# su1phurd/UAV-WRF-LES-PPO-LSTM

Hardware: AMD Instinct MI355X
Metric: env-steps/sec (rollout + GAE + 5-epoch PPO update), 4096 envs x 128 T per GPU, LSTM h=128 x1 (higher is better)
Workload: dtype f32

## Files before the change

### uav-wrf-les-ppo-lstm_amd/csrc/lstm.hip

```cpp
#include <stdlib.h>
#include <type_traits>
#include "common.h"

int gemm_f32(uav_ctx* ctx, int64_t M, int64_t N, int64_t K, const float* A, int64_t sa_m, int64_t sa_k,
             const float* B, int64_t sb_k, int64_t sb_n, float* C, int64_t ldc, const float* bias,
             int accumulate, hipStream_t st);
int colsum(uav_ctx* ctx, const float* X, int64_t B, int C, float* out, float* scratch, hipStream_t st);
int colsum_absmax(uav_ctx* ctx, const float* X, int64_t B, int C, float* out, float* scratch, unsigned* absmax_bits,
                  hipStream_t st);
int colsum_xw(uav_ctx* ctx, const float* X, int64_t B, int C, const float* x, int I, float* colsum_out, float* xw_out,
              float* scratch, unsigned* absmax_bits, hipStream_t st, int xw_transposed = 0);
bool gemm_h3_ok(int64_t M, int64_t N, int64_t K, const float* A, int64_t sa_m, int64_t sa_k, const float* B, int64_t sb_k,
                int64_t sb_n);
int gemm_h3(uav_ctx* ctx, int64_t M, int64_t N, int64_t K, const float* A, int64_t sa_m, int64_t sa_k, const float* B,
            int64_t sb_k, int64_t sb_n, float* C, int64_t ldc, const float* bias, int accumulate, const unsigned* a_absmax,
            hipStream_t st);
int lstm_generic_fwd(uav_ctx* ctx, const float* keep, const float* h0, const float* c0, const float* w_hh, int N, int T,
                     int H, float* y, float* hn, float* cn, float* stash, hipStream_t st);
int lstm_h3_fwd(uav_ctx* ctx, const float* x, int I, const float* w_ih, const float* b_ih, const float* b_hh,
                const float* keep, const float* h0, const float* c0, const float* w_hh, int N, int T, float* y, float* hn,
                float* cn, float* stash, hipStream_t st);
bool lstm_h3_step_path(int H);
int lstm_generic_bwd(uav_ctx* ctx, const float* keep, const float* stash, const float* w_hh, const float* dy,
                     const float* dheads, const float* w_head, int n_heads,
// ... 101 lines not shown
            const int t = t0 + tt;
            f32x4 acc[4];
#pragma unroll
            for (int q = 0; q < 4; ++q) {
                if (FUSE_X) {
                    acc[q] = f32x4{bias[q], bias[q], bias[q], bias[q]};
                } else {
#pragma unroll
                    for (int r = 0; r < 4; ++r) {
                        const int n = min(n0 + 4 * kq + r, N - 1);
                        acc[q][r] = stash[((size_t)n * T + t) * (6 * H) + q * H + u];
                    }
                }
            }
            if (FUSE_X) {
                const float2 ax = *reinterpret_cast<const float2*>(&xbuf[(tt * MT + j) * 8 + 2 * kq]);
#pragma unroll
                for (int q = 0; q < 4; ++q) {
                    acc[q] = __builtin_amdgcn_mfma_f32_16x16x4f32(ax.x, wx[q][0], acc[q], 0, 0, 0);
                    acc[q] = __builtin_amdgcn_mfma_f32_16x16x4f32(ax.y, wx[q][1], acc[q], 0, 0, 0);
                }
            }
            const float* hrow = hbuf + cur * MT * S + j * S + kq * SEG;
#pragma unroll
            for (int s = 0; s < KS; s += 4) {
                const float4 a = *reinterpret_cast<const float4*>(hrow + s);
#pragma unroll
                for (int q = 0; q < 4; ++q) acc[q] = __builtin_amdgcn_mfma_f32_16x16x4f32(a.x, wh[q][s], acc[q], 0, 0, 0);
#pragma unroll
                for (int q = 0; q < 4; ++q) acc[q] = __builtin_amdgcn_mfma_f32_16x16x4f32(a.y, wh[q][s + 1], acc[q], 0, 0, 0);
#pragma unroll
                for (int q = 0; q < 4; ++q) acc[q] = __builtin_amdgcn_mfma_f32_16x16x4f32(a.z, wh[q][s + 2], acc[q], 0, 0, 0);
#pragma unroll
                for (int q = 0; q < 4; ++q) acc[q] = __builtin_amdgcn_mfma_f32_16x16x4f32(a.w, wh[q][s + 3], acc[q], 0, 0, 0);
            }
            float* hnext = hbuf + (cur ^ 1) * MT * S;
#pragma unroll
            for (int r = 0; r < 4; ++r) {
                const int e = 4 * kq + r;
                const int n = n0 + e;
                const float gi = sigmoidf_(acc[0][r]), gf = sigmoidf_(acc[1][r]);
                const float gg = tanhf_(acc[2][r]), go = sigmoidf_(acc[3][r]);
                const float cp = c_reg[r];
                const float c = gf * cp + gi * gg;
                const float h = go * tanhf_(c);
                const float kn = kbuf[(tt + 1) * MT + e];
                if (n < N) {
                    const size_t row = (size_t)n * T + t;
                    y[row * H + u] = h;
                    if (stash) {
                        float* sp = stash + row * (6 * H);
                        sp[u] = gi; sp[H + u] = gf; sp[2 * H + u] = gg; sp[3 * H + u] = go;
                        sp[4 * H + u] = cp;
                        if (I > 6) sp[5 * H + u] = hin[r];
                    }
                }
                h_last[r] = h;
                if (t == T - 1) c_reg[r] = c;
                else c_reg[r] = c * kn;
                hin[r] = h * kn;
                hnext[e * S + hpos<H>(u)] = hin[r];
            }
            cur ^= 1;
            lds_barrier();
        }
    }
#pragma unroll
    for (int r = 0; r < 4; ++r) {
        const int n = n0 + 4 * kq + r;
        if (n < N) {
            hn[(size_t)n * H + u] = h_last[r];
            cn[(size_t)n * H + u] = c_reg[r];
        }
    }
}

template <class P, int H>
struct FwdSplitGeom {
    static constexpr int NS = H / 32;
    static constexpr int RS = H + 8;
    static constexpr int PLANE = MT * RS;
    static constexpr int QL = P::fwd_park(H);
    static constexpr int WPARK = QL * NS * 64 * 8;
    static constexpr int TCX = 8;
    static constexpr int XPT = (MT * TCX * 8 + H * 4 - 1) / (H * 4);
    static constexpr int HPL = 8 * RS;
    static constexpr size_t LDS = (2 * P::NP * PLANE + (H / 16) * WPARK + P::NP * HPL) * sizeof(unsigned short) +
                                  (2 * TCX * MT * 8 + 2 * TCX * MT + (H / 16) * 8 * 64 + 4 * H + 8) * sizeof(float);
};
#ifdef UAV_X6_PROFILE
__device__ unsigned long long g_x6_prof[2][8];
#define X6_PROF_DECL unsigned long long pm_[8] = {0, 0, 0, 0, 0, 0, 0, 0}, pl_ = __builtin_readcyclecounter()
#define X6_PROF_MARK(i) do { const unsigned long long n_ = __builtin_readcyclecounter(); pm_[i] += n_ - pl_; pl_ = n_; } while (0)
#define X6_PROF_DEP(v) asm volatile("" ::"v"(v))
#define X6_PROF_FLUSH() do { if (blockIdx.x == 0 && lane == 0 && (w == 0 || w == H / 16 - 1)) \
        for (int i_ = 0; i_ < 4; ++i_) g_x6_prof[w ? 1 : 0][i_] = pm_[i_]; } while (0)
#define X6_PROF_FLUSH8() do { if (blockIdx.x == 0 && lane == 0 && (w == 0 || w == H / 16 - 1)) \
        for (int i_ = 0; i_ < 8; ++i_) g_x6_prof[w ? 1 : 0][i_] = pm_[i_]; } while (0)
extern "C" int uav_x6_prof_read(unsigned long long* out) {
    return hipMemcpyFromSymbol(out, HIP_SYMBOL(g_x6_prof), sizeof(g_x6_prof)) == hipSuccess ? 0 : 1;
}
#else
#define X6_PROF_DECL
#define X6_PROF_MARK(i)
#define X6_PROF_DEP(v)
#define X6_PROF_FLUSH()
#define X6_PROF_FLUSH8()
#endif

template <class P, int H, bool FUSE_X>
__device__ __forceinline__ void lstm_fwd_split(
    const float* __restrict__ x, const float* __restrict__ keep, const float* __restrict__ h0,
    const float* __restrict__ c0, const float* __restrict__ w_ih, const float* __restrict__ w_hh,
    const float* __restrict__ b_ih, const float* __restrict__ b_hh, int N, int T, int I,
    float* __restrict__ y, float* __restrict__ hn, float* __restrict__ cn, float* __restrict__ stash,
    const float* __restrict__ w_head, const float* __restrict__ b_head, int NHD, float* __restrict__ heads) {
    using G = FwdSplitGeom<P, H>;
    using vec = typename P::vec;
    using piece = typename P::piece;
    constexpr int NP = P::NP, NS = G::NS, RS = G::RS, PLANE = G::PLANE, QL = G::QL, WPARK = G::WPARK, TC = G::TCX;
    constexpr int XPT = G::XPT, NT = H * 4, HPL = G::HPL, NW = H / 16;
    extern __shared__ __attribute__((aligned(16))) float smem[];
    unsigned short* hpl = reinterpret_cast<unsigned short*>(smem);
    unsigned short* wpark = hpl + 2 * NP * PLANE;
    float* xbuf = reinterpret_cast<float*>(wpark + (H / 16) * WPARK);
    float* kbuf = xbuf + 2 * TC * MT * 8;
    float* wxl = kbuf + 2 * TC * MT;
    float* bl = wxl + (H / 16) * 512;
    unsigned short* whp = reinterpret_cast<unsigned short*>(bl + 4 * H + 8);

    const int lane = threadIdx.x & 63, w = threadIdx.x >> 6;
    const int j = lane & 15, kq = lane >> 4;
    const int uw = 16 * w + j;
    const int uo = 16 * w + 4 * kq;
    const int n0 = blockIdx.x * MT;
    const int n = min(n0 + j, N - 1);
    const bool live = n0 + j < N;

    vec wb[4][NS][NP];
    vec* const wpk = reinterpret_cast<vec*>(wpark + w * WPARK) + lane;
#pragma unroll
    for (int q = 0; q < 4; ++q)
#pragma unroll
        for (int s = 0; s < NS; ++s) {
            const float* src = w_hh + (size_t)(q * H + uw) * H + 32 * s + 8 * kq;
            const float4 v0 = *reinterpret_cast<const float4*>(src), v1 = *reinterpret_cast<const float4*>(src + 4);
            const float v[8] = {v0.x, v0.y, v0.z, v0.w, v1.x, v1.y, v1.z, v1.w};
#pragma unroll
            for (int i = 0; i < 8; ++i) {
                piece p[NP];
                P::split(v[i], p);
#pragma unroll
                for (int pc = 0; pc < NP; ++pc) wb[q][s][pc][i] = p[pc];
            }
            if (q < QL) wpk[(q * NS + s) * 64] = wb[q][s][NP - 1];
        }
    float* const wxw = wxl + w * 512 + lane;
    if (FUSE_X) {
#pragma unroll
        for (int q = 0; q < 4; ++q)
#pragma unroll
            for (int s = 0; s < 2; ++s) {
                const int k = 2 * kq + s;
                wxw[(2 * q + s) * 64] = (k < I) ? w_ih[(size_t)(q * H + uw) * I + k] : 0.f;
            }
        for (int idx = threadIdx.x; idx < 4 * H; idx += NT) bl[idx] = b_ih[idx] + b_hh[idx];
    }
    if (heads) {
        for (int idx = threadIdx.x; idx < 8 * H; idx += NT) {
            const int hdx = idx / H, uu = idx % H;
            piece p[NP];
            P::split((hdx < NHD) ? w_head[(size_t)hdx * H + uu] : 0.f, p);
            unsigned short* d = whp + hdx * RS + uu;
#pragma unroll
            for (int pc = 0; pc < NP; ++pc) d[pc * HPL] = P::bits(p[pc]);
        }
        if (threadIdx.x < 8) bl[4 * H + threadIdx.x] = (int)threadIdx.x < NHD ? b_head[threadIdx.x] : 0.f;
    }
    auto emit_heads = [&](int buf, int t) {
        f32x4 ha = {0.f, 0.f, 0.f, 0.f}, hb = ha;
        const unsigned short* hrow = hpl + buf * NP * PLANE + j * RS + 8 * kq;
        const unsigned short* wrow = whp + (j & 7) * RS + 8 * kq;
#pragma unroll
        for (int s = 0; s < NS; ++s) {
            P::head_slab(ha, hb, [&](int pc) { return *reinterpret_cast<const vec*>(wrow + pc * HPL + 32 * s); },
                         [&](int pc) { return *reinterpret_cast<const vec*>(hrow + pc * PLANE + 32 * s); });
            asm volatile("" ::: "memory");
        }
        if (live && kq < 2) {
            float* dst = heads + ((size_t)n * T + t) * NHD;
#pragma unroll
            for (int r = 0; r < 4; ++r)
                if (4 * kq + r < NHD) dst[4 * kq + r] = P::sum(ha[r], hb[r]) + bl[4 * H + 4 * kq + r];
        }
    };
    auto put_h = [&](unsigned short* plane0, const float (&hv)[4]) {
        unsigned short b[NP][4];
#pragma unroll
        for (int r = 0; r < 4; ++r) {
            piece p[NP];
            P::split(hv[r], p);
#pragma unroll
            for (int pc = 0; pc < NP; ++pc) b[pc][r] = P::bits(p[pc]);
        }
#pragma unroll
        for (int pc = 0; pc < NP; ++pc) {
            uint2 v;
            v.x = (unsigned)b[pc][0] | ((unsigned)b[pc][1] << 16);
            v.y = (unsigned)b[pc][2] | ((unsigned)b[pc][3] << 16);
            *reinterpret_cast<uint2*>(plane0 + pc * PLANE + j * RS + uo) = v;
        }
    };

    float xr[XPT], kr = 1.f;
    auto stage_load = [&](int t0) {
        if (FUSE_X) {
#pragma unroll
            for (int i = 0; i < XPT; ++i) {
                const int idx = threadIdx.x + i * NT;
                const int e = min(idx / (TC * 8), MT - 1), tt = (idx >> 3) % TC, f = idx & 7;
                const int ne = min(n0 + e, N - 1), t = min(t0 + tt, T - 1);
                xr[i] = (f < I) ? x[((size_t)ne * T + t) * I + f] : 0.f;
            }
        }
        if (threadIdx.x < TC * MT) {
            const int e = threadIdx.x / TC, tt = threadIdx.x % TC;
            const int ne = min(n0 + e, N - 1), t = t0 + tt + 1;
            kr = (keep && t < T) ? keep[(size_t)ne * T + t] : 1.f;
        }
    };
    auto stage_commit = [&](int buf) {
        if (FUSE_X) {
#pragma unroll
            for (int i = 0; i < XPT; ++i) {
                const int idx = threadIdx.x + i * NT;
                const int e = idx / (TC * 8), tt = (idx >> 3) % TC, f = idx & 7;
                if (e < MT) xbuf[((buf * TC + tt) * MT + e) * 8 + f] = xr[i];
            }
        }
        if (threadIdx.x < TC * MT) kbuf[(buf * TC + threadIdx.x % TC) * MT + threadIdx.x / TC] = kr;
    };

    float c_reg[4];
    {
        const float k0 = keep ? keep[(size_t)n * T] : 1.f;
        const float4 cv = *reinterpret_cast<const float4*>(c0 + (size_t)n * H + uo);
        const float4 hv4 = *reinterpret_cast<const float4*>(h0 + (size_t)n * H + uo);
        c_reg[0] = cv.x * k0; c_reg[1] = cv.y * k0; c_reg[2] = cv.z * k0; c_reg[3] = cv.w * k0;
        const float hv[4] = {hv4.x * k0, hv4.y * k0, hv4.z * k0, hv4.w * k0};
        put_h(hpl, hv);
        if (stash && I > 6 && live)
            *reinterpret_cast<float4*>(stash + ((size_t)n * T) * (6 * H) + 5 * H + uo) = float4{hv[0], hv[1], hv[2], hv[3]};
    }
    stage_load(0);
    stage_commit(0);
    int cur = 0;
    float kcur = 1.f;
    X6_PROF_DECL;
    lds_barrier();

    const int nchunk = (T + TC - 1) / TC;
    for (int ch = 0; ch < nchunk; ++ch) {
        const int t0 = ch * TC, tc = min(TC, T - t0), xb = ch & 1;
        if (ch + 1 < nchunk) stage_load(t0 + TC);
        for (int tt = 0; tt < tc; ++tt) {
            const int t = t0 + tt;
            const size_t row = (size_t)n * T + t;
            X6_PROF_MARK(0);
            if (heads && w == NW - 1 && t > 0) emit_heads(cur, t - 1);
            f32x4 acc[4], acl[4];
#pragma unroll
            for (int q = 0; q < 4; ++q) acc[q] = acl[q] = f32x4{0.f, 0.f, 0.f, 0.f};
            const unsigned short* hrow = hpl + cur * NP * PLANE + j * RS + 8 * kq;
#pragma unroll
            for (int s = 0; s < NS; ++s) {
                vec a[NP];
#pragma unroll
                for (int pc = 0; pc < NP; ++pc) a[pc] = *reinterpret_cast<const vec*>(hrow + pc * PLANE + 32 * s);
                auto wf = [&](int q, int p) { return (p == NP - 1 && q < QL) ? wpk[(q * NS + s) * 64] : wb[q][s][p]; };
                P::gates_slab(acc, acl, wf, a);
            }
#pragma unroll
            for (int q = 0; q < 4; ++q) {
                const float4 v = FUSE_X ? *reinterpret_cast<const float4*>(bl + q * H + uo)
                                        : *reinterpret_cast<const float4*>(stash + row * (6 * H) + q * H + uo);
                acc[q] = P::sum(acc[q], acl[q]) * kcur + f32x4{v.x, v.y, v.z, v.w};
            }
            if (FUSE_X) {
                const float2 ax = *reinterpret_cast<const float2*>(&xbuf[((xb * TC + tt) * MT + j) * 8 + 2 * kq]);
#pragma unroll
                for (int q = 0; q < 4; ++q) {
                    acc[q] = __builtin_amdgcn_mfma_f32_16x16x4f32(wxw[(2 * q) * 64], ax.x, acc[q], 0, 0, 0);
                    acc[q] = __builtin_amdgcn_mfma_f32_16x16x4f32(wxw[(2 * q + 1) * 64], ax.y, acc[q], 0, 0, 0);
                }
            }
            X6_PROF_DEP(acc[0][0]); X6_PROF_DEP(acc[1][1]); X6_PROF_DEP(acc[2][2]); X6_PROF_DEP(acc[3][3]);
            X6_PROF_MARK(1);
            const float kn = kbuf[(xb * TC + tt) * MT + j];
            float gi[4], gf[4], gg[4], go[4], cp[4], hh[4], hm[4], cc[4];
            float* sp = stash + row * (6 * H) + uo;
#pragma unroll
            for (int r = 0; r < 4; ++r) {
                gi[r] = sigmoidf_(acc[0][r]); gf[r] = sigmoidf_(acc[1][r]); gg[r] = tanhf_(acc[2][r]);
                cp[r] = c_reg[r];
                cc[r] = H >= 128 ? __builtin_fmaf(gi[r], gg[r], gf[r] * cp[r])
                                 : __builtin_fmaf(gf[r], cp[r], gi[r] * gg[r]);
            }
            if (live && stash) {
                *reinterpret_cast<float4*>(sp) = float4{gi[0], gi[1], gi[2], gi[3]};
                *reinterpret_cast<float4*>(sp + H) = float4{gf[0], gf[1], gf[2], gf[3]};
                *reinterpret_cast<float4*>(sp + 2 * H) = float4{gg[0], gg[1], gg[2], gg[3]};
                *reinterpret_cast<float4*>(sp + 4 * H) = float4{cp[0], cp[1], cp[2], cp[3]};
            }
#pragma unroll
            for (int r = 0; r < 4; ++r) {
                go[r] = sigmoidf_(acc[3][r]);
                hh[r] = go[r] * tanhf_(cc[r]);
                hm[r] = hh[r] * kn;
                c_reg[r] = (t == T - 1) ? cc[r] : cc[r] * kn;
            }
            put_h(hpl + (cur ^ 1) * NP * PLANE, hh);
            kcur = kn;
            if (live) {
                *reinterpret_cast<float4*>(y + row * H + uo) = float4{hh[0], hh[1], hh[2], hh[3]};
                if (stash) {
                    *reinterpret_cast<float4*>(sp + 3 * H) = float4{go[0], go[1], go[2], go[3]};
                    if (I > 6 && t + 1 < T)
                        *reinterpret_cast<float4*>(sp + 6 * H + 5 * H) = float4{hm[0], hm[1], hm[2], hm[3]};
                }
                if (t == T - 1) {
                    *reinterpret_cast<float4*>(hn + (size_t)n * H + uo) = float4{hh[0], hh[1], hh[2], hh[3]};
                    *reinterpret_cast<float4*>(cn + (size_t)n * H + uo) = float4{c_reg[0], c_reg[1], c_reg[2], c_reg[3]};
                }
            }
            cur ^= 1;
            X6_PROF_MARK(2);
            lds_barrier();
            X6_PROF_MARK(3);
        }
        if (ch + 1 < nchunk) {
            stage_commit(xb ^ 1);
            lds_barrier();
        }
    }
    if (heads && w == NW - 1) emit_heads(cur, T - 1);
    X6_PROF_FLUSH();
}

template <int H, bool FUSE_X>
__global__ __launch_bounds__(H * 4) void lstm_fwd_h3_kernel(
    const float* __restrict__ x, const float* __restrict__ keep, const float* __restrict__ h0,
    const float* __restrict__ c0, const float* __restrict__ w_ih, const float* __restrict__ w_hh,
    const float* __restrict__ b_ih, const float* __restrict__ b_hh, int N, int T, int I,
    float* __restrict__ y, float* __restrict__ hn, float* __restrict__ cn, float* __restrict__ stash,
    const float* __restrict__ w_head, const float* __restrict__ b_head, int NHD, float* __restrict__ heads) {
    lstm_fwd_split<SplitF16x3, H, FUSE_X>(x, keep, h0, c0, w_ih, w_hh, b_ih, b_hh, N, T, I, y, hn, cn, stash, w_head,
                                          b_head, NHD, heads);
}
template <int H, bool FUSE_X>
__global__ __launch_bounds__(H * 4) void lstm_fwd_x6_kernel(
    const float* __restrict__ x, const float* __restrict__ keep, const float* __restrict__ h0,
    const float* __restrict__ c0, const float* __restrict__ w_ih, const float* __restrict__ w_hh,
    const float* __restrict__ b_ih, const float* __restrict__ b_hh, int N, int T, int I,
    float* __restrict__ y, float* __restrict__ hn, float* __restrict__ cn, float* __restrict__ stash,
    const float* __restrict__ w_head, const float* __restrict__ b_head, int NHD, float* __restrict__ heads) {
    lstm_fwd_split<SplitBf16x6, H, FUSE_X>(x, keep, h0, c0, w_ih, w_hh, b_ih, b_hh, N, T, I, y, hn, cn, stash, w_head,
                                           b_head, NHD, heads);
}

template <int H>
struct BwdGeom {
    static constexpr int S = 4 * H + 4;
    static constexpr size_t LDS = (2 * MT * S + TC * MT * 8 + (TC + 1) * MT) * sizeof(float);
};

template <int H>
__global__ __launch_bounds__(H * 4) void lstm_bwd_kernel(
    const float* __restrict__ keep, const float* __restrict__ stash, const float* __restrict__ w_hh,
    const float* __restrict__ dy, const float* __restrict__ dheads, const float* __restrict__ w_head, int NH,
    const float* __restrict__ dhn, const float* __restrict__ dcn, int N, int T, float* __restrict__ dgates,
    float* __restrict__ dh0, float* __restrict__ dc0) {
    using G = BwdGeom<H>;
    constexpr int S = G::S;
    extern __shared__ __attribute__((aligned(16))) float smem[];
    float* dgbuf = smem;
    float* dhbuf = dgbuf + 2 * MT * S;
    float* kbuf = dhbuf + TC * MT * 8;

    const int lane = threadIdx.x & 63, w = threadIdx.x >> 6;
    const int j = lane & 15, kq = lane >> 4;
    const int u = 16 * w + j;
    const int n0 = blockIdx.x * MT;

    float wt[H];
#pragma unroll
    for (int s = 0; s < H; ++s) wt[s] = w_hh[(size_t)(kq * H + s) * H + u];
    float whb[2];
#pragma unroll
    for (int a = 0; a < 2; ++a) whb[a] = (dheads && 4 * a + kq < NH) ? w_head[(size_t)(4 * a + kq) * H + u] : 0.f;

    float dh_rec[4], dc_next[4];
    size_t srow[4];
#pragma unroll
    for (int r = 0; r < 4; ++r) {
        const int n = min(n0 + 4 * kq + r, N - 1);
        dh_rec[r] = dhn ? dhn[(size_t)n * H + u] : 0.f;
        dc_next[r] = dcn ? dcn[(size_t)n * H + u] : 0.f;
        srow[r] = (size_t)n * T;
    }
    float pf[4][5], pdy[4];
    auto prefetch = [&](int t) {
#pragma unroll
        for (int r = 0; r < 4; ++r) {
            const float* sp = stash + (srow[r] + t) * (6 * H);
            pf[r][0] = sp[u]; pf[r][1] = sp[H + u]; pf[r][2] = sp[2 * H + u]; pf[r][3] = sp[3 * H + u];
            pf[r][4] = sp[4 * H + u];
            pdy[r] = dy ? dy[(srow[r] + t) * H + u] : 0.f;
        }
    };
    prefetch(T - 1);
    int cur = 0;
    const int nchunk = (T + TC - 1) / TC;
    for (int ch = nchunk - 1; ch >= 0; --ch) {
        const int t0 = ch * TC, tc = min(TC, T - t0);
        if (dheads) {
            for (int idx = threadIdx.x; idx < MT * tc * 8; idx += blockDim.x) {
                const int e = idx / (tc * 8), rem = idx % (tc * 8), tt = rem >> 3, f = rem & 7;
                const int n = min(n0 + e, N - 1);
                dhbuf[(tt * MT + e) * 8 + f] = (f < NH) ? dheads[((size_t)n * T + t0 + tt) * NH + f] : 0.f;
            }
        }
        for (int idx = threadIdx.x; idx < MT * tc; idx += blockDim.x) {
            const int e = idx / tc, tt = idx % tc;
            const int n = min(n0 + e, N - 1);
            kbuf[tt * MT + e] = keep ? keep[(size_t)n * T + t0 + tt] : 1.f;
        }
        lds_barrier();
        for (int tt = tc - 1; tt >= 0; --tt) {
            const int t = t0 + tt;
            float* dgw = dgbuf + cur * MT * S;
            f32x4 dyacc = {0.f, 0.f, 0.f, 0.f};
            if (dheads) {
                const float* dr = &dhbuf[(tt * MT + j) * 8];
                dyacc = __builtin_amdgcn_mfma_f32_16x16x4f32(dr[kq], whb[0], dyacc, 0, 0, 0);
                dyacc = __builtin_amdgcn_mfma_f32_16x16x4f32(dr[4 + kq], whb[1], dyacc, 0, 0, 0);
            }
#pragma unroll
            for (int r = 0; r < 4; ++r) {
                const int e = 4 * kq + r;
                const float gi = pf[r][0], gf = pf[r][1], gg = pf[r][2], go = pf[r][3], cp = pf[r][4];
// ... 35 lines not shown
                dh_rec[r] = ((a0[r] + a1[r]) + (a2[r] + a3[r])) * kp;
            }
            cur ^= 1;
        }
        lds_barrier();
    }
#pragma unroll
    for (int r = 0; r < 4; ++r) {
        const int n = n0 + 4 * kq + r;
        if (n < N) {
            if (dh0) dh0[(size_t)n * H + u] = dh_rec[r];
            if (dc0) dc0[(size_t)n * H + u] = dc_next[r];
        }
    }
}

template <class P, int H>
struct BwdSplitGeom {
    static constexpr int NW = H / 16;
    static constexpr int SLOT = 5 * MT * 16;
    static constexpr int SMALL = 128;
    static constexpr int PK = P::bwd_park(H);
    static constexpr int WPARK = PK * 64 * 8;
    static constexpr size_t LDS = (NW * NW * 64 * 4  + NW * SLOT + 2 * SMALL) * sizeof(float) +
                                  NW * WPARK * sizeof(unsigned short);
};

template <class P, int H>
__device__ __forceinline__ void lstm_bwd_split(
    const float* __restrict__ keep, const float* __restrict__ stash, const float* __restrict__ w_hh,
    const float* __restrict__ dheads, const float* __restrict__ w_head, int NH, const float* __restrict__ dhn,
    const float* __restrict__ dcn, int N, int T, float* __restrict__ dgates, float* __restrict__ dh0,
    float* __restrict__ dc0) {
    using G = BwdSplitGeom<P, H>;
    using vec = typename P::vec;
    using piece = typename P::piece;
    constexpr int NP = P::NP, SLOT = G::SLOT, NW = G::NW, SMALL = G::SMALL, PK = G::PK, WPARK = G::WPARK;
    extern __shared__ __attribute__((aligned(16))) float smem[];
    f32x4* part = reinterpret_cast<f32x4*>(smem);
    float* ring = smem + NW * NW * 64 * 4;
    float* small = ring + NW * SLOT;
    unsigned short* wpark = reinterpret_cast<unsigned short*>(small + 2 * SMALL);

    const int lane = threadIdx.x & 63;
    const int w = __builtin_amdgcn_readfirstlane(threadIdx.x >> 6);
    const int j = lane & 15, kq = lane >> 4;
    const int uw = 16 * w + j;
    const int uo = 16 * w + 4 * kq;
    const int n0 = blockIdx.x * MT;
    const int n = min(n0 + j, N - 1);
    const bool live = n0 + j < N;

    vec wa[NW][2][NP];
    vec* const wpk = reinterpret_cast<vec*>(wpark + w * WPARK) + lane;
#pragma unroll
    for (int m = 0; m < NW; ++m)
#pragma unroll
        for (int sb = 0; sb < 2; ++sb) {
#pragma unroll
            for (int e = 0; e < 8; ++e) {
                const int k = (2 * sb + e / 4) * H + 16 * w + 4 * kq + (e % 4);
                piece p[NP];
                P::split(w_hh[(size_t)k * H + 16 * m + j], p);
#pragma unroll
                for (int pc = 0; pc < NP; ++pc) wa[m][sb][pc][e] = p[pc];
            }
            if (2 * m + sb < PK) wpk[(2 * m + sb) * 64] = wa[m][sb][NP - 1];
        }
    float whb[2];
#pragma unroll
    for (int a = 0; a < 2; ++a) whb[a] = (4 * a + kq < NH) ? w_head[(size_t)(4 * a + kq) * H + uw] : 0.f;

    float dh_rec[4], dc_next[4];
    {
        const float4 a4 = dhn ? *reinterpret_cast<const float4*>(dhn + (size_t)n * H + uo) : float4{0.f, 0.f, 0.f, 0.f};
        const float4 c4 = dcn ? *reinterpret_cast<const float4*>(dcn + (size_t)n * H + uo) : float4{0.f, 0.f, 0.f, 0.f};
        dh_rec[0] = a4.x; dh_rec[1] = a4.y; dh_rec[2] = a4.z; dh_rec[3] = a4.w;
        dc_next[0] = c4.x; dc_next[1] = c4.y; dc_next[2] = c4.z; dc_next[3] = c4.w;
    }
    const size_t srow = (size_t)n * T;

    typedef __attribute__((address_space(3))) float lds_f;
    const int e_d = lane >> 2, g4 = lane & 3;
    const size_t drow = (size_t)min(n0 + e_d, N - 1) * T;
    const unsigned ring_base = __builtin_amdgcn_readfirstlane((unsigned)(unsigned long)((lds_f*)(ring + w * SLOT)));
    const unsigned small_base = __builtin_amdgcn_readfirstlane((unsigned)(unsigned long)((lds_f*)small));
    auto issue = [&](int t) {
        const float* src = stash + (drow + t) * (6 * H) + 16 * w + 4 * g4;
        unsigned m0save;
        asm volatile(
            "s_mov_b32 %0, m0\n\t"
            "s_mov_b32 m0, %6\n\ts_nop 0\n\tglobal_load_lds_dwordx4 %1, off\n\t"
            "s_add_u32 m0, m0, 1024\n\ts_nop 0\n\tglobal_load_lds_dwordx4 %2, off\n\t"
            "s_add_u32 m0, m0, 1024\n\ts_nop 0\n\tglobal_load_lds_dwordx4 %3, off\n\t"
            "s_add_u32 m0, m0, 1024\n\ts_nop 0\n\tglobal_load_lds_dwordx4 %4, off\n\t"
            "s_add_u32 m0, m0, 1024\n\ts_nop 0\n\tglobal_load_lds_dwordx4 %5, off\n\t"
            "s_mov_b32 m0, %0"
            : "=&s"(m0save)
            : "v"(src), "v"(src + H), "v"(src + 2 * H), "v"(src + 3 * H), "v"(src + 4 * H), "s"(ring_base)
            : "memory", "scc");
    };
    const float* small_at0;
    unsigned small_stride;
    {
        const int e = w * 64 + lane;
        if (e < 16 * NH) { small_at0 = dheads + (size_t)min(n0 + e / NH, N - 1) * T * NH + e % NH; small_stride = (unsigned)NH; }
        else if (e >= 112 && keep) { small_at0 = keep + (size_t)min(n0 + e - 112, N - 1) * T; small_stride = 1u; }
        else { small_at0 = w_hh + (lane & 15); small_stride = 0u; }
    }
    auto issue_small = [&](int t, int slot) {
        const float* src = small_at0 + (size_t)((unsigned)t * small_stride);
        const unsigned dst = small_base + (unsigned)((slot * SMALL + w * 64) * 4);
        unsigned m0save;
        asm volatile("s_mov_b32 %0, m0\n\ts_mov_b32 m0, %2\n\ts_nop 0\n\tglobal_load_lds_dword %1, off\n\ts_mov_b32 m0, %0"
                     : "=&s"(m0save) : "v"(src), "s"(dst) : "memory");
    };
    const bool small_wave = w < 2;
    issue(T - 1);
    if (small_wave) {
        issue_small(T - 1, (T - 1) & 1);
        issue_small(T >= 2 ? T - 2 : 0, (T - 2) & 1);
    }
    bool first = true;
    X6_PROF_DECL;
    for (int t = T - 1; t >= 0; --t) {
        X6_PROF_MARK(0);
        if (first) asm volatile("s_waitcnt vmcnt(0)" ::: "memory");
        else if (small_wave) asm volatile("s_waitcnt vmcnt(5)" ::: "memory");
        else asm volatile("s_waitcnt vmcnt(4)" ::: "memory");
        first = false;
        const float* sl = ring + w * SLOT + j * 16 + 4 * kq;
        float4 pf[5];
#pragma unroll
        for (int q = 0; q < 5; ++q) pf[q] = *reinterpret_cast<const float4*>(sl + q * 256);
        asm volatile("s_waitcnt lgkmcnt(0)" ::: "memory");
        issue(t >= 1 ? t - 1 : 0);
        X6_PROF_MARK(1);
        lds_barrier();
        X6_PROF_MARK(2);
        const float* sm = small + (t & 1) * SMALL;
        f32x4 dyacc = {0.f, 0.f, 0.f, 0.f};
        {
            const float d0 = (kq < NH) ? sm[j * NH + kq] : 0.f;
            const float d1 = (4 + kq < NH) ? sm[j * NH + 4 + kq] : 0.f;
            dyacc = __builtin_amdgcn_mfma_f32_16x16x4f32(whb[0], d0, dyacc, 0, 0, 0);
            dyacc = __builtin_amdgcn_mfma_f32_16x16x4f32(whb[1], d1, dyacc, 0, 0, 0);
        }
        const float kp = keep ? sm[112 + j] : 1.f;
        const float gi[4] = {pf[0].x, pf[0].y, pf[0].z, pf[0].w}, gf[4] = {pf[1].x, pf[1].y, pf[1].z, pf[1].w};
        const float gg[4] = {pf[2].x, pf[2].y, pf[2].z, pf[2].w}, go[4] = {pf[3].x, pf[3].y, pf[3].z, pf[3].w};
        const float cp[4] = {pf[4].x, pf[4].y, pf[4].z, pf[4].w};
        float dg[4][4];
#pragma unroll
        for (int r = 0; r < 4; ++r) {
            const float dh = dyacc[r] + dh_rec[r];
            const float c = __builtin_fmaf(gf[r], cp[r], gi[r] * gg[r]);
            const float tch = tanhf_(c);
            const float dc = dh * go[r] * (1.0f - tch * tch) + dc_next[r];
            dg[0][r] = dc * gg[r] * gi[r] * (1.0f - gi[r]);
            dg[1][r] = dc * cp[r] * gf[r] * (1.0f - gf[r]);
            dg[2][r] = dc * gi[r] * (1.0f - gg[r] * gg[r]);
            dg[3][r] = dh * tch * go[r] * (1.0f - go[r]);
            dc_next[r] = dc * gf[r] * kp;
        }
        int ex = 0;
        float unscale = 1.f;
        if constexpr (P::BLOCK_SCALE) {
            float mx = 0.f;
#pragma unroll
            for (int q = 0; q < 4; ++q)
#pragma unroll
                for (int r = 0; r < 4; ++r) mx = fmaxf(mx, fabsf(dg[q][r]));
            {
                const unsigned u = __builtin_bit_cast(unsigned, mx);
                const auto s16 = __builtin_amdgcn_permlane16_swap(u, u, false, false);
                mx = fmaxf(__builtin_bit_cast(float, (unsigned)s16[0]), __builtin_bit_cast(float, (unsigned)s16[1]));
                const unsigned v = __builtin_bit_cast(unsigned, mx);
                const auto s32 = __builtin_amdgcn_permlane32_swap(v, v, false, false);
                mx = fmaxf(__builtin_bit_cast(float, (unsigned)s32[0]), __builtin_bit_cast(float, (unsigned)s32[1]));
            }
            ex = 14 - __builtin_amdgcn_frexp_expf(mx);
            ex = mx > 0.f ? min(max(ex, -100), 100) : 0;
// ... 10 lines not shown
                piece p[NP];
                P::split(P::BLOCK_SCALE ? __builtin_amdgcn_ldexpf(dg[q][r], ex) : dg[q][r], p);
#pragma unroll
                for (int pc = 0; pc < NP; ++pc) bp[q >> 1][pc][4 * (q & 1) + r] = p[pc];
            }
            if constexpr (!P::DG_STORES_LATE) store_dg(q);
        }
        X6_PROF_DEP(bp[1][NP - 1]); X6_PROF_DEP(bp[0][0]);
        X6_PROF_MARK(3);
#pragma unroll
        for (int m = 0; m < NW; ++m) {
            f32x4 a0 = {0.f, 0.f, 0.f, 0.f}, a1 = a0;
#pragma unroll
            for (int sb = 0; sb < 2; ++sb) {
                const int item = 2 * m + sb;
                P::tile_slab(a0, a1, [&](int p) { return (p == NP - 1 && item < PK) ? wpk[item * 64] : wa[m][sb][p]; }, bp[sb]);
            }
            part[(m * NW + w) * 64 + lane] = P::tile_sum(a0, a1) * unscale;
        }
        if constexpr (P::DG_STORES_LATE) {
#pragma unroll
            for (int q = 0; q < 4; ++q) store_dg(q);
        }
        asm volatile("s_waitcnt lgkmcnt(0)" ::: "memory");
        X6_PROF_MARK(4);
        lds_barrier();
        X6_PROF_MARK(5);
        if (small_wave) issue_small(t >= 2 ? t - 2 : 0, t & 1);
        f32x4 sum = part[(w * NW) * 64 + lane];
#pragma unroll
        for (int ww = 1; ww < NW; ++ww) sum += part[(w * NW + ww) * 64 + lane];
#pragma unroll
        for (int r = 0; r < 4; ++r) dh_rec[r] = sum[r] * kp;
        X6_PROF_DEP(dh_rec[3]);
        X6_PROF_MARK(6);
    }
    X6_PROF_FLUSH8();
    asm volatile("s_waitcnt vmcnt(0)" ::: "memory");
    if (live) {
        if (dh0) *reinterpret_cast<float4*>(dh0 + (size_t)n * H + uo) = float4{dh_rec[0], dh_rec[1], dh_rec[2], dh_rec[3]};
        if (dc0) *reinterpret_cast<float4*>(dc0 + (size_t)n * H + uo) = float4{dc_next[0], dc_next[1], dc_next[2], dc_next[3]};
    }
}

template <int H>
__global__ __launch_bounds__(H * 4) void lstm_bwd_h3k_kernel(
    const float* __restrict__ keep, const float* __restrict__ stash, const float* __restrict__ w_hh,
    const float* __restrict__ dheads, const float* __restrict__ w_head, int NH, const float* __restrict__ dhn,
    const float* __restrict__ dcn, int N, int T, float* __restrict__ dgates, float* __restrict__ dh0,
    float* __restrict__ dc0) {
    lstm_bwd_split<SplitF16x3, H>(keep, stash, w_hh, dheads, w_head, NH, dhn, dcn, N, T, dgates, dh0, dc0);
}
template <int H>
__global__ __launch_bounds__(H * 4) void lstm_bwd_x6k_kernel(
    const float* __restrict__ keep, const float* __restrict__ stash, const float* __restrict__ w_hh,
    const float* __restrict__ dheads, const float* __restrict__ w_head, int NH, const float* __restrict__ dhn,
    const float* __restrict__ dcn, int N, int T, float* __restrict__ dgates, float* __restrict__ dh0,
    float* __restrict__ dc0) {
    lstm_bwd_split<SplitBf16x6, H>(keep, stash, w_hh, dheads, w_head, NH, dhn, dcn, N, T, dgates, dh0, dc0);
}

template <class P, int H, bool FUSE_X>
static constexpr auto fwd_split_kernel() {
    if constexpr (std::is_same<P, SplitF16x3>::value) return &lstm_fwd_h3_kernel<H, FUSE_X>;
    else return &lstm_fwd_x6_kernel<H, FUSE_X>;
}
template <class P, int H>
static constexpr auto bwd_split_kernel() {
    if constexpr (std::is_same<P, SplitF16x3>::value) return &lstm_bwd_h3k_kernel<H>;
    else return &lstm_bwd_x6k_kernel<H>;
}

template <class F>
static int with_split(F&& f) {
    return uav_want_bf16x6() ? f(SplitBf16x6{}) : f(SplitF16x3{});
}

template <class P, int H>
static int launch_bwd_split(const float* keep, const float* stash, const float* w_hh, const float* dheads,
                            const float* w_head, int NH, const float* dhn, const float* dcn, int N, int T, float* dgates,
                            float* dh0, float* dc0, hipStream_t st) {
    const dim3 grid((N + MT - 1) / MT), block(H * 4);
    const size_t lx = BwdSplitGeom<P, H>::LDS;
    constexpr auto kern = bwd_split_kernel<P, H>();
    UAV_CHECK_HIP(uav_dyn_lds(reinterpret_cast<const void*>(kern), (int)lx));
    hipLaunchKernelGGL(kern, grid, block, lx, st, keep, stash, w_hh, dheads, w_head, NH, dhn, dcn, N, T, dgates, dh0, dc0);
    UAV_LAUNCH_CHECK();
    return 0;
}

template <class P, int H>
static int launch_fwd_split(bool fuse, const float* x, const float* keep, const float* h0, const float* c0,
                            const float* w_ih, const float* w_hh, const float* b_ih, const float* b_hh, int N, int T, int I,
                            float* y, float* hn, float* cn, float* stash, const float* w_head, const float* b_head, int NHD,
                            float* heads, hipStream_t st) {
    const dim3 grid((N + MT - 1) / MT), block(H * 4);
    const size_t lx = FwdSplitGeom<P, H>::LDS;
    constexpr auto fused = fwd_split_kernel<P, H, true>(), unfused = fwd_split_kernel<P, H, false>();
    UAV_CHECK_HIP(uav_dyn_lds(reinterpret_cast<const void*>(fused), (int)lx));
    UAV_CHECK_HIP(uav_dyn_lds(reinterpret_cast<const void*>(unfused), (int)lx));
    hipLaunchKernelGGL(fuse ? fused : unfused, grid, block, lx, st, x, keep, h0, c0, w_ih, w_hh, b_ih, b_hh, N, T, I, y, hn,
                       cn, stash, w_head, b_head, NHD, heads);
    UAV_LAUNCH_CHECK();
    return 0;
}

template <int H>
static int launch_fwd(bool fuse, const float* x, const float* keep, const float* h0, const float* c0,
                      const float* w_ih, const float* w_hh, const float* b_ih, const float* b_hh, int N, int T, int I,
                      float* y, float* hn, float* cn, float* stash, const float* w_head, const float* b_head, int NHD,
                      float* heads, bool* heads_done, hipStream_t st) {
    if (!uav_want_f32_mfma()) {
        *heads_done = heads != nullptr;
        return with_split([&](auto p) {
            return launch_fwd_split<decltype(p), H>(fuse, x, keep, h0, c0, w_ih, w_hh, b_ih, b_hh, N, T, I, y, hn, cn, stash,
                                                    w_head, b_head, NHD, heads, st);
        });
    }
    const dim3 grid((N + MT - 1) / MT), block(H * 4);
    const size_t lds = FwdGeom<H>::LDS;
    if (fuse)
        hipLaunchKernelGGL((lstm_fwd_kernel<H, true>), grid, block, lds, st, x, keep, h0, c0, w_ih, w_hh, b_ih, b_hh, N,
                           T, I, y, hn, cn, stash);
    else
        hipLaunchKernelGGL((lstm_fwd_kernel<H, false>), grid, block, lds, st, x, keep, h0, c0, w_ih, w_hh, b_ih, b_hh,
                           N, T, I, y, hn, cn, stash);
    UAV_LAUNCH_CHECK();
    return 0;
}

template <int H>
static int launch_bwd(const float* keep, const float* stash, const float* w_hh, const float* dy, const float* dheads,
                      const float* w_head, int NH, const float* dhn, const float* dcn, int N, int T, float* dgates,
                      float* dh0, float* dc0, hipStream_t st) {
    const dim3 grid((N + MT - 1) / MT), block(H * 4);
    UAV_CHECK_HIP(uav_dyn_lds(reinterpret_cast<const void*>(&lstm_bwd_kernel<H>), (int)BwdGeom<H>::LDS));
    hipLaunchKernelGGL((lstm_bwd_kernel<H>), grid, block, BwdGeom<H>::LDS, st, keep, stash, w_hh, dy, dheads, w_head, NH,
                       dhn, dcn, N, T, dgates, dh0, dc0);
    UAV_LAUNCH_CHECK();
    return 0;
}

__global__ void add2_kernel(const float* a0, const float* a1, float* b, int n) {
    const int i = blockIdx.x * 256 + threadIdx.x;
    if (i < n) b[i] = a0[i] + a1[i];
}

static int lstm_bwd_seq(const float* keep, const float* stash, const float* w_hh, const float* dy,
                        const float* dheads, const float* w_head, int NH, const float* dhn, const float* dcn, int N,
                        int T, int H, float* dgates, float* dh0, float* dc0, hipStream_t st) {
    if (dheads && NH <= 7 && !uav_want_f32_mfma()) {
        return with_split([&](auto p) {
            using P = decltype(p);
            return H == 64 ? launch_bwd_split<P, 64>(keep, stash, w_hh, dheads, w_head, NH, dhn, dcn, N, T, dgates, dh0, dc0, st)
                           : launch_bwd_split<P, 128>(keep, stash, w_hh, dheads, w_head, NH, dhn, dcn, N, T, dgates, dh0, dc0, st);
        });
    }
    switch (H) {
        case 64: return launch_bwd<64>(keep, stash, w_hh, dy, dheads, w_head, NH, dhn, dcn, N, T, dgates, dh0, dc0, st);
        case 128: return launch_bwd<128>(keep, stash, w_hh, dy, dheads, w_head, NH, dhn, dcn, N, T, dgates, dh0, dc0, st);
    }
    uav_set_error("uav_lstm_bwd: H=%d unsupported (64, 128)", H);
    return 2;
}

extern "C" {

int uav_lstm_fwd(uav_ctx* ctx, const float* x, const float* keep, const float* h0, const float* c0, const float* w_ih,
                 const float* w_hh, const float* b_ih, const float* b_hh, int N, int T, int I, int H, float* y,
                 float* hn, float* cn, float* stash, const float* w_head, const float* b_head, int n_heads, float* heads,
                 uav_stream stream) {
    UAV_REQUIRE(ctx && x && h0 && c0 && w_ih && w_hh && b_ih && b_hh && y && hn && cn, "uav_lstm_fwd: NULL argument");
    uav_enter(ctx);
    UAV_REQUIRE(N > 0 && T > 0 && I > 0, "uav_lstm_fwd: N=%d T=%d I=%d", N, T, I);
    UAV_REQUIRE(!heads || (w_head && b_head && n_heads > 0 && n_heads <= 8), "uav_lstm_fwd: heads needs w_head, b_head, 1..8 heads");
    hipStream_t st = as_stream(stream);
    const bool persistent = (H == 64 || H == 128);
    const bool fuse = I <= 8 && persistent;
    const bool step256 = lstm_h3_step_path(H);
    if (step256) UAV_REQUIRE(stash, "uav_lstm_fwd: stash is required when H is not 64/128");
    if (!fuse && !step256) {
        UAV_REQUIRE(stash, "uav_lstm_fwd: stash is required when I > 8 or H is not 64/128");
        float* bsum = (float*)ctx->ws;
        uav_ctx sub = *ctx;
        sub.ws = (char*)ctx->ws + 65536;
// ... 158 lines not shown
```

Baseline: 75.73 million.

## Stage whole x/keep sequence into LDS via async DMA in LSTM forward

Replaces the 8-step register-staged double buffer for x and keep in the split-precision LSTM forward with global_load_lds DMA that stages up to 128 timesteps into a large LDS image, sized per T at launch. This removes per-chunk register load/commit phases and the barriers between them, at the cost of much more LDS per workgroup, which can lower occupancy. It also vectorises head stores for NHD=6. In the backward kernel, per-lane 64-bit stash addresses become scalar base plus 32-bit offsets, with new T limit checks to guard against overflow.

```diff
diff --git a/uav-wrf-les-ppo-lstm_amd/csrc/lstm.hip b/uav-wrf-les-ppo-lstm_amd/csrc/lstm.hip
--- a/uav-wrf-les-ppo-lstm_amd/csrc/lstm.hip
+++ b/uav-wrf-les-ppo-lstm_amd/csrc/lstm.hip
@@ -207,12 +207,18 @@
     static constexpr int PLANE = MT * RS;
     static constexpr int QL = P::fwd_park(H);
     static constexpr int WPARK = QL * NS * 64 * 8;
-    static constexpr int TCX = 8;
-    static constexpr int XPT = (MT * TCX * 8 + H * 4 - 1) / (H * 4);
     static constexpr int HPL = 8 * RS;
-    static constexpr size_t LDS = (2 * P::NP * PLANE + (H / 16) * WPARK + P::NP * HPL) * sizeof(unsigned short) +
-                                  (2 * TCX * MT * 8 + 2 * TCX * MT + (H / 16) * 8 * 64 + 4 * H + 8) * sizeof(float);
+    static constexpr size_t FIXED = (2 * P::NP * PLANE + (H / 16) * WPARK + P::NP * HPL) * sizeof(unsigned short) +
+                                    ((H / 16) * 8 * 64 + 4 * H + 8) * sizeof(float);
+    static constexpr size_t STEP = MT * (8 + 1) * sizeof(float);
+    static constexpr size_t LDS_CAP = (H >= 128 ? 160 : 80) * 1024;
+    static constexpr int TS_MAX = (int)((LDS_CAP - FIXED) / STEP) / 8 * 8 < 128 ? (int)((LDS_CAP - FIXED) / STEP) / 8 * 8 : 128;
+    static_assert(TS_MAX >= 8, "lstm_fwd_split: no LDS left for the x / keep image");
+    static constexpr size_t lds_bytes(int ts) { return FIXED + (size_t)ts * STEP; }
+    static_assert(FIXED + (size_t)TS_MAX * STEP <= LDS_CAP, "lstm_fwd_split: the fullest x / keep image exceeds the LDS budget");
 };
+template <class G>
+static int fwd_split_steps(int T) { return T <= G::TS_MAX ? (T + 3) / 4 * 4 : G::TS_MAX; }
 #ifdef UAV_X6_PROFILE
 __device__ unsigned long long g_x6_prof[2][8];
 #define X6_PROF_DECL unsigned long long pm_[8] = {0, 0, 0, 0, 0, 0, 0, 0}, pl_ = __builtin_readcyclecounter()
@@ -239,20 +245,20 @@
     const float* __restrict__ c0, const float* __restrict__ w_ih, const float* __restrict__ w_hh,
     const float* __restrict__ b_ih, const float* __restrict__ b_hh, int N, int T, int I,
     float* __restrict__ y, float* __restrict__ hn, float* __restrict__ cn, float* __restrict__ stash,
-    const float* __restrict__ w_head, const float* __restrict__ b_head, int NHD, float* __restrict__ heads) {
+    const float* __restrict__ w_head, const float* __restrict__ b_head, int NHD, float* __restrict__ heads, int TS) {
     using G = FwdSplitGeom<P, H>;
     using vec = typename P::vec;
     using piece = typename P::piece;
-    constexpr int NP = P::NP, NS = G::NS, RS = G::RS, PLANE = G::PLANE, QL = G::QL, WPARK = G::WPARK, TC = G::TCX;
-    constexpr int XPT = G::XPT, NT = H * 4, HPL = G::HPL, NW = H / 16;
+    constexpr int NP = P::NP, NS = G::NS, RS = G::RS, PLANE = G::PLANE, QL = G::QL, WPARK = G::WPARK;
+    constexpr int NT = H * 4, HPL = G::HPL, NW = H / 16;
     extern __shared__ __attribute__((aligned(16))) float smem[];
     unsigned short* hpl = reinterpret_cast<unsigned short*>(smem);
     unsigned short* wpark = hpl + 2 * NP * PLANE;
-    float* xbuf = reinterpret_cast<float*>(wpark + (H / 16) * WPARK);
-    float* kbuf = xbuf + 2 * TC * MT * 8;
-    float* wxl = kbuf + 2 * TC * MT;
+    float* wxl = reinterpret_cast<float*>(wpark + (H / 16) * WPARK);
     float* bl = wxl + (H / 16) * 512;
     unsigned short* whp = reinterpret_cast<unsigned short*>(bl + 4 * H + 8);
+    float* xbuf = reinterpret_cast<float*>(whp + NP * HPL);
+    float* kbuf = xbuf + TS * MT * 8;
 
     const int lane = threadIdx.x & 63, w = threadIdx.x >> 6;
     const int j = lane & 15, kq = lane >> 4;
@@ -262,6 +268,30 @@
     const int n = min(n0 + j, N - 1);
     const bool live = n0 + j < N;
 
+    typedef __attribute__((address_space(3))) float lds_f;
+    const int ws = __builtin_amdgcn_readfirstlane(threadIdx.x >> 6);
+    const unsigned xbuf_lds = __builtin_amdgcn_readfirstlane((unsigned)(unsigned long)((lds_f*)xbuf));
+    const unsigned kbuf_lds = __builtin_amdgcn_readfirstlane((unsigned)(unsigned long)((lds_f*)kbuf));
+    const float* const x_tile = x + (size_t)n0 * T * I;
+    const float* const k_tile = keep ? keep + (size_t)n0 * T : w_hh;
+    const unsigned x_lane = ((unsigned)min(8 * (ws & 1) + (lane >> 3), N - 1 - n0) * T * I + ((lane & 7) < I ? (lane & 7) : 0)) * 4u;
+    const unsigned k_lane = keep ? (unsigned)min(lane & 15, N - 1 - n0) * T * 4u : (unsigned)lane * 4u;
+    const unsigned k_step = keep ? 4u : 0u;
+    auto dma = [&](const float* ubase, unsigned off_bytes, unsigned lds_dst) {
+        unsigned m0save;
+        asm volatile("s_mov_b32 %0, m0\n\ts_mov_b32 m0, %3\n\ts_nop 0\n\tglobal_load_lds_dword %1, %2\n\ts_mov_b32 m0, %0"
+                     : "=&s"(m0save) : "v"(off_bytes), "s"(ubase), "s"(lds_dst) : "memory");
+    };
+    auto stage = [&](int t0, int slot0, int ns) {
+        if (FUSE_X)
+            for (int s = ws >> 1; s < ns; s += NW / 2)
+                dma(x_tile, x_lane + (unsigned)min(t0 + s, T - 1) * (unsigned)(I * 4), xbuf_lds + (unsigned)((2 * (slot0 + s) + (ws & 1)) * 256));
+        for (int p = ws; 4 * p < ns; p += NW)
+            dma(k_tile, k_lane + (unsigned)min(t0 + 4 * p + (lane >> 4) + 1, T - 1) * k_step, kbuf_lds + (unsigned)((slot0 + 4 * p) * 64));
+    };
+    const int HS = T <= TS ? TS : TS / 2;
+    stage(0, 0, HS);
+
     vec wb[4][NS][NP];
     vec* const wpk = reinterpret_cast<vec*>(wpark + w * WPARK) + lane;
 #pragma unroll
@@ -314,9 +344,16 @@
         }
         if (live && kq < 2) {
             float* dst = heads + ((size_t)n * T + t) * NHD;
-#pragma unroll
-            for (int r = 0; r < 4; ++r)
-                if (4 * kq + r < NHD) dst[4 * kq + r] = P::sum(ha[r], hb[r]) + bl[4 * H + 4 * kq + r];
+            if (NHD == 6) {
+                const float4 b4 = *reinterpret_cast<const float4*>(bl + 4 * H + 4 * kq);
+                const f32x4 hs = P::sum(ha, hb);
+                *reinterpret_cast<float2*>(dst + 4 * kq) = float2{hs[0] + b4.x, hs[1] + b4.y};
+                if (kq == 0) *reinterpret_cast<float2*>(dst + 2) = float2{hs[2] + b4.z, hs[3] + b4.w};
+            } else {
+#pragma unroll
+                for (int r = 0; r < 4; ++r)
+                    if (4 * kq + r < NHD) dst[4 * kq + r] = P::sum(ha[r], hb[r]) + bl[4 * H + 4 * kq + r];
+            }
         }
     };
     auto put_h = [&](unsigned short* plane0, const float (&hv)[4]) {
@@ -335,35 +372,6 @@
             v.y = (unsigned)b[pc][2] | ((unsigned)b[pc][3] << 16);
             *reinterpret_cast<uint2*>(plane0 + pc * PLANE + j * RS + uo) = v;
         }
-    };
-
-    float xr[XPT], kr = 1.f;
-    auto stage_load = [&](int t0) {
-        if (FUSE_X) {
-#pragma unroll
-            for (int i = 0; i < XPT; ++i) {
-                const int idx = threadIdx.x + i * NT;
-                const int e = min(idx / (TC * 8), MT - 1), tt = (idx >> 3) % TC, f = idx & 7;
-                const int ne = min(n0 + e, N - 1), t = min(t0 + tt, T - 1);
-                xr[i] = (f < I) ? x[((size_t)ne * T + t) * I + f] : 0.f;
-            }
-        }
-        if (threadIdx.x < TC * MT) {
-            const int e = threadIdx.x / TC, tt = threadIdx.x % TC;
-            const int ne = min(n0 + e, N - 1), t = t0 + tt + 1;
-            kr = (keep && t < T) ? keep[(size_t)ne * T + t] : 1.f;
-        }
-    };
-    auto stage_commit = [&](int buf) {
-        if (FUSE_X) {
-#pragma unroll
-            for (int i = 0; i < XPT; ++i) {
-                const int idx = threadIdx.x + i * NT;
-                const int e = idx / (TC * 8), tt = (idx >> 3) % TC, f = idx & 7;
-                if (e < MT) xbuf[((buf * TC + tt) * MT + e) * 8 + f] = xr[i];
-            }
-        }
-        if (threadIdx.x < TC * MT) kbuf[(buf * TC + threadIdx.x % TC) * MT + threadIdx.x / TC] = kr;
     };
 
     float c_reg[4];
@@ -377,17 +385,16 @@
         if (stash && I > 6 && live)
             *reinterpret_cast<float4*>(stash + ((size_t)n * T) * (6 * H) + 5 * H + uo) = float4{hv[0], hv[1], hv[2], hv[3]};
     }
-    stage_load(0);
-    stage_commit(0);
     int cur = 0;
     float kcur = 1.f;
     X6_PROF_DECL;
+    asm volatile("s_waitcnt vmcnt(0)" ::: "memory");
     lds_barrier();
 
-    const int nchunk = (T + TC - 1) / TC;
-    for (int ch = 0; ch < nchunk; ++ch) {
-        const int t0 = ch * TC, tc = min(TC, T - t0), xb = ch & 1;
-        if (ch + 1 < nchunk) stage_load(t0 + TC);
+    const int nfill = (T + HS - 1) / HS;
+    for (int ch = 0; ch < nfill; ++ch) {
+        const int t0 = ch * HS, tc = min(HS, T - t0), sb = (ch & 1) * HS;
+        if (ch + 1 < nfill) stage(t0 + HS, sb ^ HS, HS);
         for (int tt = 0; tt < tc; ++tt) {
             const int t = t0 + tt;
             const size_t row = (size_t)n * T + t;
@@ -412,7 +419,7 @@
                 acc[q] = P::sum(acc[q], acl[q]) * kcur + f32x4{v.x, v.y, v.z, v.w};
             }
             if (FUSE_X) {
-                const float2 ax = *reinterpret_cast<const float2*>(&xbuf[((xb * TC + tt) * MT + j) * 8 + 2 * kq]);
+                const float2 ax = *reinterpret_cast<const float2*>(&xbuf[((sb + tt) * MT + j) * 8 + 2 * kq]);
 #pragma unroll
                 for (int q = 0; q < 4; ++q) {
                     acc[q] = __builtin_amdgcn_mfma_f32_16x16x4f32(wxw[(2 * q) * 64], ax.x, acc[q], 0, 0, 0);
@@ -421,7 +428,8 @@
             }
             X6_PROF_DEP(acc[0][0]); X6_PROF_DEP(acc[1][1]); X6_PROF_DEP(acc[2][2]); X6_PROF_DEP(acc[3][3]);
             X6_PROF_MARK(1);
-            const float kn = kbuf[(xb * TC + tt) * MT + j];
+            const float ks = kbuf[(sb + tt) * MT + j];
+            const float kn = (keep && t + 1 < T) ? ks : 1.f;
             float gi[4], gf[4], gg[4], go[4], cp[4], hh[4], hm[4], cc[4];
             float* sp = stash + row * (6 * H) + uo;
 #pragma unroll
@@ -463,8 +471,8 @@
             lds_barrier();
             X6_PROF_MARK(3);
         }
-        if (ch + 1 < nchunk) {
-            stage_commit(xb ^ 1);
+        if (ch + 1 < nfill) {
+            asm volatile("s_waitcnt vmcnt(0)" ::: "memory");
             lds_barrier();
         }
     }
@@ -478,9 +486,9 @@
     const float* __restrict__ c0, const float* __restrict__ w_ih, const float* __restrict__ w_hh,
     const float* __restrict__ b_ih, const float* __restrict__ b_hh, int N, int T, int I,
     float* __restrict__ y, float* __restrict__ hn, float* __restrict__ cn, float* __restrict__ stash,
-    const float* __restrict__ w_head, const float* __restrict__ b_head, int NHD, float* __restrict__ heads) {
+    const float* __restrict__ w_head, const float* __restrict__ b_head, int NHD, float* __restrict__ heads, int TS) {
     lstm_fwd_split<SplitF16x3, H, FUSE_X>(x, keep, h0, c0, w_ih, w_hh, b_ih, b_hh, N, T, I, y, hn, cn, stash, w_head,
-                                          b_head, NHD, heads);
+                                          b_head, NHD, heads, TS);
 }
 template <int H, bool FUSE_X>
 __global__ __launch_bounds__(H * 4) void lstm_fwd_x6_kernel(
@@ -488,9 +496,9 @@
     const float* __restrict__ c0, const float* __restrict__ w_ih, const float* __restrict__ w_hh,
     const float* __restrict__ b_ih, const float* __restrict__ b_hh, int N, int T, int I,
     float* __restrict__ y, float* __restrict__ hn, float* __restrict__ cn, float* __restrict__ stash,
-    const float* __restrict__ w_head, const float* __restrict__ b_head, int NHD, float* __restrict__ heads) {
+    const float* __restrict__ w_head, const float* __restrict__ b_head, int NHD, float* __restrict__ heads, int TS) {
     lstm_fwd_split<SplitBf16x6, H, FUSE_X>(x, keep, h0, c0, w_ih, w_hh, b_ih, b_hh, N, T, I, y, hn, cn, stash, w_head,
-                                           b_head, NHD, heads);
+                                           b_head, NHD, heads, TS);
 }
 
 template <int H>
@@ -692,22 +700,23 @@
 
     typedef __attribute__((address_space(3))) float lds_f;
     const int e_d = lane >> 2, g4 = lane & 3;
-    const size_t drow = (size_t)min(n0 + e_d, N - 1) * T;
+    const float* const s_tile = stash + (size_t)n0 * T * (6 * H);
+    const unsigned d_lane = ((unsigned)min(e_d, N - 1 - n0) * T * (6 * H) + 16 * w + 4 * g4) * 4u;
     const unsigned ring_base = __builtin_amdgcn_readfirstlane((unsigned)(unsigned long)((lds_f*)(ring + w * SLOT)));
     const unsigned small_base = __builtin_amdgcn_readfirstlane((unsigned)(unsigned long)((lds_f*)small));
     auto issue = [&](int t) {
-        const float* src = stash + (drow + t) * (6 * H) + 16 * w + 4 * g4;
+        const unsigned off = d_lane + (unsigned)t * (unsigned)(6 * H * 4);
         unsigned m0save;
         asm volatile(
             "s_mov_b32 %0, m0\n\t"
-            "s_mov_b32 m0, %6\n\ts_nop 0\n\tglobal_load_lds_dwordx4 %1, off\n\t"
-            "s_add_u32 m0, m0, 1024\n\ts_nop 0\n\tglobal_load_lds_dwordx4 %2, off\n\t"
-            "s_add_u32 m0, m0, 1024\n\ts_nop 0\n\tglobal_load_lds_dwordx4 %3, off\n\t"
-            "s_add_u32 m0, m0, 1024\n\ts_nop 0\n\tglobal_load_lds_dwordx4 %4, off\n\t"
-            "s_add_u32 m0, m0, 1024\n\ts_nop 0\n\tglobal_load_lds_dwordx4 %5, off\n\t"
+            "s_mov_b32 m0, %7\n\ts_nop 0\n\tglobal_load_lds_dwordx4 %1, %2\n\t"
+            "s_add_u32 m0, m0, 1024\n\ts_nop 0\n\tglobal_load_lds_dwordx4 %1, %3\n\t"
+            "s_add_u32 m0, m0, 1024\n\ts_nop 0\n\tglobal_load_lds_dwordx4 %1, %4\n\t"
+            "s_add_u32 m0, m0, 1024\n\ts_nop 0\n\tglobal_load_lds_dwordx4 %1, %5\n\t"
+            "s_add_u32 m0, m0, 1024\n\ts_nop 0\n\tglobal_load_lds_dwordx4 %1, %6\n\t"
             "s_mov_b32 m0, %0"
             : "=&s"(m0save)
-            : "v"(src), "v"(src + H), "v"(src + 2 * H), "v"(src + 3 * H), "v"(src + 4 * H), "s"(ring_base)
+            : "v"(off), "s"(s_tile), "s"(s_tile + H), "s"(s_tile + 2 * H), "s"(s_tile + 3 * H), "s"(s_tile + 4 * H), "s"(ring_base)
             : "memory", "scc");
     };
     const float* small_at0;
@@ -884,6 +893,7 @@
                             float* dh0, float* dc0, hipStream_t st) {
     const dim3 grid((N + MT - 1) / MT), block(H * 4);
     const size_t lx = BwdSplitGeom<P, H>::LDS;
+    UAV_REQUIRE((int64_t)T * 6 * H < ((int64_t)1 << 26), "uav_lstm_bwd: T=%d is beyond the h = %d sequence kernel's 32-bit tile offsets (T 6H < 2^26)", T, H);
     constexpr auto kern = bwd_split_kernel<P, H>();
     UAV_CHECK_HIP(uav_dyn_lds(reinterpret_cast<const void*>(kern), (int)lx));
     hipLaunchKernelGGL(kern, grid, block, lx, st, keep, stash, w_hh, dheads, w_head, NH, dhn, dcn, N, T, dgates, dh0, dc0);
@@ -897,12 +907,16 @@
                             float* y, float* hn, float* cn, float* stash, const float* w_head, const float* b_head, int NHD,
                             float* heads, hipStream_t st) {
     const dim3 grid((N + MT - 1) / MT), block(H * 4);
-    const size_t lx = FwdSplitGeom<P, H>::LDS;
+    using G = FwdSplitGeom<P, H>;
+    UAV_REQUIRE(T < (1 << 23), "uav_lstm_fwd: T=%d is beyond the h = 64 / 128 sequence kernel's 32-bit tile offsets (T < 2^23)", T);
+    const int ts = fwd_split_steps<G>(T);
+    const size_t lx = G::lds_bytes(ts);
+    UAV_REQUIRE(lx <= 160 * 1024, "uav_lstm_fwd: %zu bytes of LDS for %d staged steps at H=%d exceed the 160 KB of a workgroup", lx, ts, H);
     constexpr auto fused = fwd_split_kernel<P, H, true>(), unfused = fwd_split_kernel<P, H, false>();
-    UAV_CHECK_HIP(uav_dyn_lds(reinterpret_cast<const void*>(fused), (int)lx));
-    UAV_CHECK_HIP(uav_dyn_lds(reinterpret_cast<const void*>(unfused), (int)lx));
+    UAV_CHECK_HIP(uav_dyn_lds(reinterpret_cast<const void*>(fused), (int)G::lds_bytes(G::TS_MAX)));
+    UAV_CHECK_HIP(uav_dyn_lds(reinterpret_cast<const void*>(unfused), (int)G::lds_bytes(G::TS_MAX)));
     hipLaunchKernelGGL(fuse ? fused : unfused, grid, block, lx, st, x, keep, h0, c0, w_ih, w_hh, b_ih, b_hh, N, T, I, y, hn,
-                       cn, stash, w_head, b_head, NHD, heads);
+                       cn, stash, w_head, b_head, NHD, heads, ts);
     UAV_LAUNCH_CHECK();
     return 0;
 }
```

Result: no change. 76.40 million (median of 6 runs) (+0.9%).
